# drowe67/pirip

Hardware: AMD Instinct MI355X
Metric: IQ Msamples/s demodulated (2-FSK Fs=240k Rs=10k); BER vs CPU ref (higher is better)
Workload: dtype f32

## Files before the change

### pirip_amd/csrc/fsk_demod_wave.hip

```cpp
#include <hip/hip_runtime.h>

#include <cmath>
#include <cstdio>
#include <cstdlib>
#include <type_traits>

#include "../../include/pirip_hip.h"
#include "demod_simd.hpp"
#include "fsk_device.hpp"

namespace pirip {

namespace {

constexpr int kWave = 64;

struct cf { float x, y; };

__device__ __forceinline__ float add_lane_up(float a, float b)
{
    float r;
    asm("v_add_f32_dpp %0, %1, %2 wave_shl:1 row_mask:0xf bank_mask:0xf bound_ctrl:0" : "=v"(r) : "v"(a), "v"(b));
    return r;
}
// ... 8 lines not shown
__device__ __forceinline__ float ubyte2(uint32_t v) { return (float)((v >> 16) & 0xffu); }
__device__ __forceinline__ float ubyte3(uint32_t v) { return (float)(v >> 24); }

__device__ __forceinline__ float llr_frame_gain_quick(int llr_map, float sig, float nse)
{
    const float a2 = sig - nse;
    if (!(a2 >= 0x1p-96f && a2 <= 0x1p126f)) return llr_frame_gain(llr_map, sig, nse);
    const float amp = sqrt_rn_normal<false>(a2);
    if (llr_map == kLlrRician) return (2.0f * amp) / nse;
    return (2.0f * (sig / nse)) / amp;
}
__device__ __forceinline__ unsigned sqrt_key(float x) { return __builtin_bit_cast(unsigned, x) - 1u; }
constexpr unsigned kSqrtLo = 0x0f800000u;
constexpr unsigned kQuickHi = 0x7c000000u;
__device__ __forceinline__ unsigned umin2(unsigned a, unsigned b) { return a < b ? a : b; }
__device__ __forceinline__ unsigned umin3(unsigned a, unsigned b, unsigned c)
{
    unsigned r;
    asm("v_min3_u32 %0, %1, %2, %3" : "=v"(r) : "v"(a), "v"(b), "v"(c));
    return r;
}

__device__ __forceinline__ v2f scale_lo(v2f h, v2f x)
{
    v2f r; asm("v_pk_mul_f32 %0, %1, %2 op_sel_hi:[0,1]" : "=v"(r) : "v"(h), "v"(x)); return r;
}
__device__ __forceinline__ v2f scale_hi(v2f h, v2f x)
{
    v2f r; asm("v_pk_mul_f32 %0, %1, %2 op_sel:[1,0] op_sel_hi:[1,1]" : "=v"(r) : "v"(h), "v"(x)); return r;
}
__device__ __forceinline__ float mag2(v2f w)
{
    v2f sq;
    asm("v_pk_mul_f32 %0, %1, %1" : "=v"(sq) : "v"(w));
    float r;
    asm("v_add_f32 %0, %1, %2" : "=v"(r) : "v"(sq.x), "v"(sq.y));
    return r;
}
__device__ __forceinline__ v2f smooth2(v2f sf, v2f mag, v2f k)
{
    v2f t;
    asm("v_pk_mul_f32 %0, %0, %3 op_sel_hi:[1,0]\n\t"
        "v_pk_mul_f32 %1, %2, %3 op_sel:[0,1] op_sel_hi:[1,1]\n\t"
        "v_pk_add_f32 %0, %0, %1"
        : "+v"(sf), "=&v"(t) : "v"(mag), "v"(k));
    return sf;
}

template <int B>
__device__ __forceinline__ uint32_t flag_mask_at(uint32_t flags)
{
    uint32_t r;
    asm("v_bfe_i32 %0, %1, %2, 1" : "=v"(r) : "v"(flags), "n"(B));
    return r;
}
__device__ __forceinline__ uint32_t flag_mask(uint32_t flags, int b)
{
    switch (b) {
    case 0: return flag_mask_at<0>(flags); case 1: return flag_mask_at<1>(flags); case 2: return flag_mask_at<2>(flags);
    case 3: return flag_mask_at<3>(flags); case 4: return flag_mask_at<4>(flags); case 5: return flag_mask_at<5>(flags);
    case 6: return flag_mask_at<6>(flags); default: return flag_mask_at<7>(flags);
    }
}

template <int FMT> struct InFmt;
template <> struct InFmt<PIRIP_IN_CU8_FSKDEMOD> { static constexpr int BPS = 2; static constexpr bool NEUTRAL_OK = true; static constexpr uint32_t NEUTRAL = 0x7F7F7F7Fu; };
template <> struct InFmt<PIRIP_IN_CU8_CSDR> { static constexpr int BPS = 2; static constexpr bool NEUTRAL_OK = false; static constexpr uint32_t NEUTRAL = 0x80808080u; };
template <> struct InFmt<PIRIP_IN_CS16> { static constexpr int BPS = 4; static constexpr bool NEUTRAL_OK = true; static constexpr uint32_t NEUTRAL = 0u; };
template <> struct InFmt<PIRIP_IN_CF32> { static constexpr int BPS = 8; static constexpr bool NEUTRAL_OK = true; static constexpr uint32_t NEUTRAL = 0u; };

__device__ __forceinline__ float cvt_s16(float x)
{
    const float hi = x * 0.00133514404296875f;
    return __builtin_fmaf(x, -0x1.e60f04p-20f, hi);
}
template <int FMT>
__device__ __forceinline__ v2f decode(const uint32_t *rw, int k)
{
    if (FMT == PIRIP_IN_CU8_FSKDEMOD || FMT == PIRIP_IN_CU8_CSDR) {
        const uint32_t v = rw[k >> 1];
        return cvt_u8_pair<FMT>(v2f{(k & 1) ? ubyte2(v) : ubyte0(v), (k & 1) ? ubyte3(v) : ubyte1(v)});
    } else if (FMT == PIRIP_IN_CS16) {
        const uint32_t v = rw[k];
        return v2f{cvt_s16((float)(short)(v & 0xffffu)), cvt_s16((float)((int)v >> 16))};
    } else {
        return v2f{__builtin_bit_cast(float, rw[2 * k]), __builtin_bit_cast(float, rw[2 * k + 1])};
    }
}
template <int FMT>
__device__ __forceinline__ v2f lds_sample(const unsigned char *p)
{
    if (FMT == PIRIP_IN_CU8_FSKDEMOD || FMT == PIRIP_IN_CU8_CSDR) {
        const uint32_t v = *(const uint16_t *)p;
        return cvt_u8_pair<FMT>(v2f{ubyte0(v), ubyte1(v)});
    } else if (FMT == PIRIP_IN_CS16) {
        const uint32_t v = *(const uint32_t *)p;
        return v2f{cvt_s16((float)(short)(v & 0xffffu)), cvt_s16((float)((int)v >> 16))};
    } else {
        const float2 v = *(const float2 *)p;
        return v2f{v.x, v.y};
    }
}

constexpr int cmax(int a, int b) { return a > b ? a : b; }

__device__ __forceinline__ float atan2_turns(float y, float x)
// ... 49 lines not shown
    static constexpr int NMEM = N + 2 * TS;
    static constexpr int Q = TS / 4;
    static constexpr int HIST = 2 * TS + Q;
    static constexpr int STEP = TS / P;
    static constexpr int NLANES = NSYM + 2;
    static constexpr int NFFT = (N - Q) / (NDFT / 2) - 1;
    static constexpr int GUARD_B = ((HIST * BPS + 15) / 16) * 16;
    static constexpr int SUP_B = (N + Q) * BPS;
    static constexpr int NDMA16 = SUP_B / 1024;
    static constexpr int NDMA4 = (SUP_B - NDMA16 * 1024 + 255) / 256;
    static constexpr bool DIRECT = FMT == PIRIP_IN_CF32 && NDFT >= 256;
    static constexpr int HEAD_B = 1024, DUMP_B = 256;
    static_assert(!DIRECT || ((TS + Q) * BPS <= HEAD_B && 3 * TS >= 2 * TS + Q), "the head holds blocks 0..2's new samples");
    static constexpr int RAW_B = DIRECT ? GUARD_B + HEAD_B + DUMP_B : GUARD_B + NDMA16 * 1024 + NDMA4 * 256;
    static constexpr int XPS256 = 16 * 17 * 8;
    static constexpr int XP_FFT_B = NDFT == 256 ? 4 * XPS256 : NDFT == 512 ? 4480 : 8 * 72 * 8;
    static constexpr int XP_B = cmax(cmax(XP_FFT_B, NDFT * 4), NDFT == 256 ? 64 * 20 * 4 : NDFT == 128 ? 8 * 136 * 4 : 0);
    static constexpr int TAIL_DW = HIST * BPS / 4;
    static constexpr int TRAILER_DW = GUARD_B / 4;
    static_assert((HIST * BPS) % 4 == 0 && (GUARD_B - HIST * BPS) % 4 == 0, "tail copies move whole dwords");
    static_assert(GUARD_B + (2 * M + 1) * 4 <= M * HIST * 8, "the state block holds the raw tail and its trailer");
    static constexpr int CHS = (BPS == 2) ? TS : (TS % 8 == 0 ? 8 : TS % 4 == 0 ? 4 : 2);
    static constexpr int CH_DW = CHS * BPS / 4;
    static_assert(TS % 2 == 0 && TS % P == 0 && P >= 4, "bad Ts / P");
    static_assert(NLANES <= kWave, "one lane per symbol block");
    static_assert((TS * BPS) % 16 == 0 && (CHS * BPS) % 16 == 0 && TS % CHS == 0, "block and chunk strides keep 16-byte alignment");
    static_assert((N + Q) / (NDFT / 2) - 1 == NFFT && N / (NDFT / 2) - 1 == NFFT, "numffts must not depend on nin");
    static_assert(NDFT == 256 ? (NFFT >= 4) : NDFT == 512 ? (NFFT % 2 == 0) : (NDFT == 128 && NFFT <= 8),
                  "FFT batches (Ndft = 256: the last batch of 4 may be partial; Ndft = 128: one batch of up to eight)");
    static_assert((NFFT - 1) * (NDFT / 2) + NDFT <= N - Q, "FFT windows stay inside the shortest frame");
    static_assert(M * P <= 48, "window prefix sums are kept in registers");
};

constexpr bool wave_plain_instance(int M, int TS, int P, int NDFT, int FMT, int WPS, bool FFT_FMA, bool MASK, int BAND)
{
    if (MASK && M == 4) return true;
    if (MASK && M == 2 && TS == 24 && FMT == PIRIP_IN_CU8_CSDR) return true;
    if (!MASK && M == 4 && FMT == PIRIP_IN_CF32 && (TS == 18 || TS == 10)) return true;
    return false;
}

constexpr bool wave_two_pass_argmax_instance(int M, int TS, int FMT, bool MASK, int BAND)
{
    if (MASK && M == 2 && TS == 24) return true;
    if (!MASK && M == 4 && (FMT == PIRIP_IN_CF32 || FMT == PIRIP_IN_CS16 || BAND == 4)) return true;
    return false;
}

constexpr bool wave_locked_paths_instance(int M, int TS, int P, int NDFT, int FMT, bool FFT_FMA, bool MASK, int BAND)
{
    return M == 2 && TS == 24 && P == 24 && NDFT == 256 && FMT == PIRIP_IN_CU8_FSKDEMOD && !FFT_FMA && !MASK && BAND == 0;
}

constexpr bool wave_packed_power_instance(int M, int TS, int P, int NDFT, int FMT, bool FFT_FMA, bool MASK, int BAND)
{
    return M == 2 && TS == 24 && P == 24 && NDFT == 256 && FMT == PIRIP_IN_CU8_FSKDEMOD && !FFT_FMA && !MASK;
}

constexpr bool wave_tail_prio_instance(int M, int TS, int P, int NDFT, int FMT, int WPS, bool FFT_FMA, bool MASK, int BAND)
{
    if (TS == 40 && M == 2 && FMT == PIRIP_IN_CS16 && !MASK) return false;
    if (TS == 40 && M == 4 && FMT == PIRIP_IN_CF32 && MASK) return false;
    if (TS == 8 && M == 2 && !MASK) return false;
    return true;
}

template <class C, int M> constexpr int wave_lds_bytes() { return C::RAW_B + C::XP_B; }

}

template <int M, int TS, int P, int NSYM, int NDFT, int FMT, int WPB, int WPS, bool FFT_FMA = false, bool MASK = false, int BAND = 0>
__global__ __launch_bounds__(kWave * WPB, WPS) void fsk_demod_wave_kernel(DemodArgs a_kernarg, int nstreams)
{
    constexpr bool INPLACE = TS == 10;
    constexpr bool PLAIN = wave_plain_instance(M, TS, P, NDFT, FMT, WPS, FFT_FMA, MASK, BAND);
    constexpr bool ARGMAX_SINGLE = !PLAIN && !wave_two_pass_argmax_instance(M, TS, FMT, MASK, BAND);
    constexpr bool TAIL_PRIO = wave_tail_prio_instance(M, TS, P, NDFT, FMT, WPS, FFT_FMA, MASK, BAND);
    constexpr bool PACKED_POWER = wave_packed_power_instance(M, TS, P, NDFT, FMT, FFT_FMA, MASK, BAND);
    static_assert(offsetof(DemodArgs, d) == 0, "the argument block is the first kernel argument");
    auto ap = [&]() {
        if constexpr (INPLACE) return (const __attribute__((address_space(4))) DemodArgs *)__builtin_amdgcn_kernarg_segment_ptr();
        else return (const DemodArgs *)&a_kernarg;
    }();
#define PIRIP_ARGS_REREAD() do { if constexpr (INPLACE) asm volatile("" : "+s"(ap)); } while (0)
#define a (*ap)
#define d (ap->d)
    static_assert(BAND == 0 || ((BAND == 2 || BAND == 4) && NDFT == 256 && !MASK), "band-only estimator: Ndft = 256, peak method, 32 or 64 bins");
    auto cmul = [](v2f x, v2f t) { return FFT_FMA ? rot_step(x, t) : cmul_x(x, t); };
    using C = WaveCfg<M, TS, P, NSYM, NDFT, FMT>;
    constexpr int N = C::N, NMEM = C::NMEM, HIST = C::HIST, STEP = C::STEP, Q = C::Q, BPS = C::BPS;
    constexpr int GUARD_B = C::GUARD_B;

    __shared__ __attribute__((aligned(16))) unsigned char s_raw[WPB][C::RAW_B];
    __shared__ __attribute__((aligned(16))) unsigned char s_xp[WPB][C::XP_B];
    constexpr int TAB_F = NDFT == 256 ? 12 * 16 * 4 : NDFT == 512 ? 8 * 16 * 2 + 12 * 32 * 2 : 8 * 16 * 2;
    __shared__ __attribute__((aligned(16))) float s_tab[TAB_F];
    __shared__ __attribute__((aligned(16))) float2 s_tph[P];
    __shared__ __attribute__((aligned(16))) float2 s_tgain[NSYM + 2];
    __shared__ float s_misc[WPB][3];
    extern __shared__ __attribute__((aligned(16))) float s_lnI0[];

    const int lane0 = threadIdx.x & (kWave - 1);
    const int wv = __builtin_amdgcn_readfirstlane(threadIdx.x >> 6);
    const int sid = blockIdx.x * WPB + wv;

    if (NDFT == 256) {
        for (int i = threadIdx.x; i < 12 * 16; i += kWave * WPB)
            ((float4 *)s_tab)[i] = ((const float4 *)a.t.fast_tab)[(i & 15) * 12 + (i >> 4)];
    } else {
        for (int i = threadIdx.x; i < TAB_F / 4; i += kWave * WPB) ((float4 *)s_tab)[i] = ((const float4 *)(a.t.fast_tab + NDFT))[i];
    }
    if constexpr (P <= 10) if (a.io.soft.llr) {
        if (a.io.soft.llr_map == kLlrRician) { for (int i = threadIdx.x; i < 258; i += kWave * WPB) s_lnI0[i] = a.io.soft.lnI0[i]; }
        else if (threadIdx.x < 20) {
            const int sg = threadIdx.x >> 2, cc = threadIdx.x & 3;
            const float c2 = sg == 0 ? 0.226f : sg == 1 ? 0.1245f : sg == 2 ? 0.0288f : sg == 3 ? 0.002f : 0.0f;
            const float c1 = sg == 0 ? 0.0125f : sg == 1 ? 0.2177f : sg == 2 ? 0.6314f : sg == 3 ? 0.9048f : 0.9867f;
            const float c0 = sg == 0 ? -0.0012f : sg == 1 ? -0.108f : sg == 2 ? -0.5645f : sg == 3 ? -1.2997f : -2.2053f;
            s_lnI0[threadIdx.x] = cc == 0 ? c2 : cc == 1 ? c1 : cc == 2 ? c0 : 0.0f;
        }
    }
    if (threadIdx.x < P) s_tph[threadIdx.x] = a.t.tph[threadIdx.x];
    if (threadIdx.x < NSYM + 2) s_tgain[threadIdx.x] = a.t.timing_rec[(threadIdx.x < NSYM + 1 ? threadIdx.x : 0) * P];
    __syncthreads();
    if (sid >= nstreams) return;
    if (a.io.seg && a.io.seg[sid].max_frames < 0) return;

    unsigned char *raw = s_raw[wv];
    unsigned char *xpb = s_xp[wv];

    uint32_t *st32 = (uint32_t *)(a.s.hist + (size_t)sid * M * HIST);
// ... 30 lines not shown

    float sc_norm_rx_timing, sc_ppm, sc_SNRest;
    int sc_nin;
    {
        const StreamScalars sc = a.s.scal[sid];
        sc_norm_rx_timing = sc.norm_rx_timing; sc_ppm = sc.ppm; sc_SNRest = sc.SNRest; sc_nin = sc.nin;
        if (lane0 == 0) { s_misc[wv][0] = sc.snr_est; s_misc[wv][1] = sc.EbNodB; s_misc[wv][2] = sc.v_est; }
    }

    int64_t seg_in = 0, out0 = 0, max_frames = a.io.max_frames;
    if (a.io.seg) {
        const SegDesc sd = a.io.seg[sid];
        seg_in = sd.in_off; out0 = sd.out_frame0; max_frames = sd.max_frames;
    }
    const uint8_t *in_base = a.io.in + (size_t)sid * a.io.in_stride + (size_t)seg_in * BPS;
    const int64_t nsamp = a.io.nsamp - seg_in;
    const __amdgpu_buffer_rsrc_t rsrc =
        __builtin_amdgcn_make_buffer_rsrc((void *)in_base, 0, (int)(uint32_t)(BPS * nsamp), 0x00020000);

    int nin = __builtin_amdgcn_readfirstlane(sc_nin);
    int64_t pos = 0, frame = 0;
    if (a.io.first) { pos = __builtin_amdgcn_readfirstlane(a.io.first[sid]); frame = pos ? 1 : 0; }
    const int64_t frame_first = frame;
    int last_freqi0 = 0, last_freqi1 = 0, last_freqi2 = 0, last_freqi3 = 0;

    uint32_t in_range = 0;
    if constexpr (!MASK && !PLAIN) {
#pragma unroll
        for (int b = 0; b < NB; b++) {
            const int sfi = (BAND && lane0 >= 16) ? -1 : own_sfi(lane0, b);
            if (sfi >= d.est_st && sfi < d.est_en) in_range |= 1u << b;
        }
    }
    constexpr bool FCACHE = WPS <= 3 && !PLAIN;
    constexpr bool KEEP_STEP = FCACHE && (M == 2 || WPS == 2);
    constexpr bool HIT_BRANCH = FCACHE && wave_locked_paths_instance(M, TS, P, NDFT, FMT, FFT_FMA, MASK, BAND);
    constexpr uint32_t kFcStale = 0x40000000u, kFcNever = 0x80000000u, kFcRan = 0x20000000u;
    static_assert(N + Q < 0x10000, "last frame's length leaves the flag bits free");
    v2f ph_c[FCACHE ? M : 1], step_c[KEEP_STEP ? M : 1];
    if constexpr (FCACHE) {
#pragma unroll
        for (int m = 0; m < M; m++) ph_c[m] = v2f{0.f, 0.f};
    }
    if constexpr (KEEP_STEP) {
#pragma unroll
        for (int m = 0; m < M; m++) step_c[m] = v2f{0.f, 0.f};
    }
    uint32_t ninp_fc = (uint32_t)ninp0 | (d.frame_cache ? kFcStale : kFcNever);
    constexpr bool LIVE_SLOTS = !PLAIN && NB == 4 && wave_locked_paths_instance(M, TS, P, NDFT, FMT, FFT_FMA, MASK, BAND);
    constexpr int NLIVE = 2;
    constexpr uint32_t kFcLowSlots = 0x10000000u;
    if constexpr (LIVE_SLOTS) {
        if (d.frame_cache && !__any((in_range >> NLIVE) != 0u)) ninp_fc |= kFcLowSlots;
    }

    typedef __attribute__((address_space(3))) void *lds_ptr;
    auto dma_frame = [&](int64_t p0) {
        const uint32_t goff = (uint32_t)__builtin_amdgcn_readfirstlane((int)(uint32_t)(p0 * BPS));
        if constexpr (C::DIRECT) {
            __builtin_amdgcn_raw_ptr_buffer_load_lds(rsrc, (lds_ptr)(raw + GUARD_B), 16, lane0 * 16, goff, 0, 0);
#pragma unroll
            for (int i = 0; i < (C::SUP_B + 8191) / 8192; i++)
                __builtin_amdgcn_raw_ptr_buffer_load_lds(rsrc, (lds_ptr)(raw + GUARD_B + C::HEAD_B), 4, lane0 * 128, goff + i * 8192, 0, 0);
            return;
        }
#pragma unroll
        for (int i = 0; i < C::NDMA16; i++)
            __builtin_amdgcn_raw_ptr_buffer_load_lds(rsrc, (lds_ptr)(raw + GUARD_B + i * 1024), 16, lane0 * 16, goff + i * 1024, 0, 0);
#pragma unroll
        for (int i = 0; i < C::NDMA4; i++)
            __builtin_amdgcn_raw_ptr_buffer_load_lds(rsrc, (lds_ptr)(raw + GUARD_B + C::NDMA16 * 1024 + i * 256), 4, lane0 * 4,
                                                     goff + C::NDMA16 * 1024 + i * 256, 0, 0);
    };
    constexpr bool SOFT_OK = P <= 10;
    uint32_t soft_carry = 0;
    int soft_cb = 0, soft_w = 0;
    uint32_t *words_o = nullptr;
    if constexpr (SOFT_OK) if (a.io.soft.llr) { words_o = a.io.soft.words + (size_t)sid * a.io.soft.words_stride + (a.io.soft.bit0 >> 5); }
    auto soft_append = [&](uint32_t W, int nb) {
        const uint32_t merged = soft_carry | (soft_cb ? (W >> soft_cb) : W);
        if (soft_cb + nb >= 32) {
            if (lane0 == 0) words_o[soft_w] = merged;
            soft_w++;
            soft_carry = soft_cb ? (W << (32 - soft_cb)) : 0u;
            soft_cb = soft_cb + nb - 32;
        } else { soft_carry = merged; soft_cb += nb; }
    };
    constexpr int NBITS = NSYM * (M == 2 ? 1 : 2);
    wave_lds_sync();
    dma_frame(pos);
    if constexpr (TAIL_PRIO) {
        auto tp = (const __attribute__((address_space(4))) DemodArgs *)__builtin_amdgcn_kernarg_segment_ptr();
        if (sid / WPB >= tp->first_tail_block) __builtin_amdgcn_s_setprio(1);
    }
    PIRIP_T_DECL;

    while (frame < max_frames && pos + nin <= nsamp) {
        PIRIP_ARGS_REREAD();
        const int nold = NMEM - nin;
        PIRIP_T_MARK(7);
        asm volatile("s_waitcnt vmcnt(0)" ::: "memory");
        wave_lds_sync();
        PIRIP_T_MARK(0);
        const unsigned char *smp = raw + GUARD_B;
        const uint32_t goff_frame = (uint32_t)__builtin_amdgcn_readfirstlane((int)(uint32_t)(pos * BPS));
        auto fft_in = [&](const unsigned char *p) -> v2f {
            if constexpr (C::DIRECT && BPS == 8) {
                const auto v = __builtin_amdgcn_raw_buffer_load_b64(rsrc, (int)(p - smp), (int)goff_frame, 0);
                return __builtin_bit_cast(v2f, v);
            } else if constexpr (C::DIRECT) {
                const uint32_t v = (uint32_t)__builtin_amdgcn_raw_buffer_load_b32(rsrc, (int)(p - smp), (int)goff_frame, 0);
                return v2f{cvt_s16((float)(short)(v & 0xffffu)), cvt_s16((float)((int)v >> 16))};
            } else return lds_sample<FMT>(p);
        };
        const v2f ktc{d.one_minus_tc, d.tc};
        if constexpr (NDFT == 256) {
            PIRIP_PHASE_LANE(lane);
            const int grp = lane >> 4, e16 = lane & 15;
            const float4 *ftab = (const float4 *)s_tab + e16;
            constexpr int XPS = C::XPS256;
            float4 tabv[12];
#pragma unroll
            for (int i = 0; i < 12; i++) tabv[i] = ftab[16 * i];
#pragma unroll 1
            for (int bt = 0; bt < (C::NFFT + 3) / 4; bt++) {
                int jj = 4 * bt + grp;
                if (C::NFFT % 4) jj = jj < C::NFFT ? jj : C::NFFT - 1;
                const int ga = e16 >> 2, gb = e16 & 3;
                const int base = ga + 4 * gb;
                const unsigned char *src = smp + BPS * ((NDFT / 2) * jj + base);
                v2f W[16];
                v2f hann2[8];
                {
                    const float4 h0 = tabv[0], h1 = tabv[1], h2 = tabv[2], h3 = tabv[3];
                    hann2[0] = v2f{h0.x, h0.y}; hann2[1] = v2f{h0.z, h0.w}; hann2[2] = v2f{h1.x, h1.y}; hann2[3] = v2f{h1.z, h1.w};
                    hann2[4] = v2f{h2.x, h2.y}; hann2[5] = v2f{h2.z, h2.w}; hann2[6] = v2f{h3.x, h3.y}; hann2[7] = v2f{h3.z, h3.w};
                }
#pragma unroll
                for (int t = 0; t < 16; t++) {
                    const v2f x = fft_in(src + 16 * BPS * t);
                    const int c = t & 3, dd = t >> 2;
                    W[4 * c + dd] = (t & 1) ? scale_hi(hann2[t >> 1], x) : scale_lo(hann2[t >> 1], x);
                }
#pragma unroll
                for (int c = 0; c < 4; c++) bfly4(W[4 * c], W[4 * c + 1], W[4 * c + 2], W[4 * c + 3]);
                bfly4(W[0], W[4], W[8], W[12]);
#pragma unroll
                for (int k = 1; k < 4; k++) {
                    v2f f1 = cmul(W[4 + k], v2f{a.tw_s2[6 * (k - 1) + 0], a.tw_s2[6 * (k - 1) + 1]});
                    v2f f2 = cmul(W[8 + k], v2f{a.tw_s2[6 * (k - 1) + 2], a.tw_s2[6 * (k - 1) + 3]});
                    v2f f3 = cmul(W[12 + k], v2f{a.tw_s2[6 * (k - 1) + 4], a.tw_s2[6 * (k - 1) + 5]});
                    bfly4(W[k], f1, f2, f3);
                    W[4 + k] = f1; W[8 + k] = f2; W[12 + k] = f3;
                }
                {
                    float2 *xp = (float2 *)(xpb + grp * XPS);
#pragma unroll
                    for (int e = 0; e < 16; e++) xp[e16 * 17 + e] = make_float2(W[e].x, W[e].y);
                    wave_lds_sync();
#pragma unroll
                    for (int g = 0; g < 16; g++) { const float2 v = xp[g * 17 + e16]; W[g] = v2f{v.x, v.y}; }
                }
                {
                    const float4 c4 = tabv[4], c5 = tabv[5];
                    const v2f tw3[3] = {v2f{c4.x, c4.y}, v2f{c4.z, c4.w}, v2f{c5.x, c5.y}};
#pragma unroll
                    for (int aa = 0; aa < 4; aa++) {
                        v2f f1 = cmul(W[4 * aa + 1], tw3[0]);
                        v2f f2 = cmul(W[4 * aa + 2], tw3[1]);
                        v2f f3 = cmul(W[4 * aa + 3], tw3[2]);
                        bfly4(W[4 * aa], f1, f2, f3);
                        W[4 * aa + 1] = f1; W[4 * aa + 2] = f2; W[4 * aa + 3] = f3;
                    }
                }
#pragma unroll
                for (int b = 0; b < (BAND ? BAND : 4); b++) {
                    const float *trow = (const float *)(ftab);
                    auto tf = [&](int f) { const float4 c = tabv[f >> 2]; return (f & 3) == 0 ? c.x : (f & 3) == 1 ? c.y : (f & 3) == 2 ? c.z : c.w; };
                    (void)trow;
                    const v2f t1{tf(22 + 6 * b), tf(23 + 6 * b)}, t2{tf(24 + 6 * b), tf(25 + 6 * b)}, t3{tf(26 + 6 * b), tf(27 + 6 * b)};
                    v2f f1 = cmul(W[4 + b], t1);
                    v2f f2 = cmul(W[8 + b], t2);
                    v2f f3 = cmul(W[12 + b], t3);
                    bfly4(W[b], f1, f2, f3);
                    W[4 + b] = f1; W[8 + b] = f2; W[12 + b] = f3;
                }
                wave_lds_sync();
                if constexpr (BAND != 0) {
                    float m2b[BAND], rb[BAND];
                    unsigned kmin = 0xffffffffu;
#pragma unroll
                    for (int b = 0; b < BAND; b++) { m2b[b] = mag2(W[b]); kmin = umin2(kmin, fbits(m2b[b])); }
                    if (__all(kmin >= kSqrtLo)) {
#pragma unroll
                        for (int b = 0; b < BAND; b++) rb[b] = sqrt_rn_normal<FMT != PIRIP_IN_CF32, true>(m2b[b]);
                    } else {
                        kmin = 0xffffffffu;
#pragma unroll
                        for (int b = 0; b < BAND; b++) kmin = umin2(kmin, sqrt_key(m2b[b]));
                        if (__all(kmin >= kSqrtLo - 1u)) {
#pragma unroll
                            for (int b = 0; b < BAND; b++) rb[b] = sqrt_rn_normal<FMT != PIRIP_IN_CF32>(m2b[b]);
                        } else {
#pragma unroll
// ... 250 lines not shown
                    for (int q0 = 0; q0 < 4; q0++) { const float2 v = x2[q0 * 40 + L5]; Y[4 * q0 + j1] = v2f{v.x, v.y}; }
                }
                float mag[16];
#pragma unroll
                for (int j1 = 0; j1 < 4; j1++) {
                    const float2 t1 = s_p3[(3 * j1 + 0) * 32 + L5], t2 = s_p3[(3 * j1 + 1) * 32 + L5], t3 = s_p3[(3 * j1 + 2) * 32 + L5];
                    v2f f0 = Y[j1];
                    v2f f1 = cmul(Y[4 + j1], v2f{t1.x, t1.y});
                    v2f f2 = cmul(Y[8 + j1], v2f{t2.x, t2.y});
                    v2f f3 = cmul(Y[12 + j1], v2f{t3.x, t3.y});
                    bfly4(f0, f1, f2, f3);
                    mag[j1] = mag2(f0); mag[j1 + 4] = mag2(f1); mag[j1 + 8] = mag2(f2); mag[j1 + 12] = mag2(f3);
                }
                float A[8], B[8];
                unsigned kmin = 0xffffffffu;
#pragma unroll
                for (int u = 0; u < 8; u++) {
                    A[u] = mag[u]; B[u] = mag[u + 8];
                    asm volatile("s_nop 1\n\tv_permlane32_swap_b32 %0, %1" : "+v"(A[u]), "+v"(B[u]));
                    kmin = umin3(kmin, fbits(A[u]), fbits(B[u]));
                }
                if (__all(kmin >= kSqrtLo)) {
#pragma unroll
                    for (int u = 0; u < 8; u++) { A[u] = sqrt_rn_normal<FMT != PIRIP_IN_CF32, true>(A[u]); B[u] = sqrt_rn_normal<FMT != PIRIP_IN_CF32, true>(B[u]); }
                } else {
                    kmin = 0xffffffffu;
#pragma unroll
                    for (int u = 0; u < 8; u++) kmin = umin3(kmin, sqrt_key(A[u]), sqrt_key(B[u]));
                    if (__all(kmin >= kSqrtLo - 1u)) {
#pragma unroll
                        for (int u = 0; u < 8; u++) { A[u] = sqrt_rn_normal<FMT != PIRIP_IN_CF32>(A[u]); B[u] = sqrt_rn_normal<FMT != PIRIP_IN_CF32>(B[u]); }
                    } else {
#pragma unroll
                        for (int u = 0; u < 8; u++) { A[u] = sqrtf(A[u]); B[u] = sqrtf(B[u]); __builtin_amdgcn_sched_barrier(0); }
                    }
                }
#pragma unroll
                for (int u = 0; u < 8; u += 2) {
                    v2f sp{Sf[u], Sf[u + 1]};
                    sp = smooth2(sp, v2f{A[u], A[u + 1]}, ktc);
                    sp = smooth2(sp, v2f{B[u], B[u + 1]}, ktc);
                    Sf[u] = sp.x; Sf[u + 1] = sp.y;
                }
                wave_lds_sync();
            }
        }

        __builtin_amdgcn_sched_barrier(0);
        PIRIP_T_MARK(1);
        int freqi[M];
#pragma unroll
        for (int m = 0; m < M; m++) freqi[m] = 0;
        int bb = 0;
        if constexpr (MASK) {
            PIRIP_PHASE_LANE(lane);
            float *sfl = (float *)xpb;
#pragma unroll
            for (int b = 0; b < NOWN; b++) sfl[own_sfi(lane, b)] = Sf[b];
            wave_lds_sync();
            float best = 0.0f; int ib = d.est_st;
            for (int b = d.est_st + lane; b < d.est_en - d.mask_len; b += kWave) {
                float corr = 0.0f;
                for (int k = 0; k < d.n_teeth; k++) corr += sfl[b + a.t.teeth[k]];
                if (corr > best) { best = corr; ib = b; }
            }
            wave_argmax<ARGMAX_SINGLE>(best, ib);
            bb = ib;
            wave_lds_sync();
        } else {
            PIRIP_PHASE_LANE(lane);
            if constexpr (LIVE_SLOTS) {
                const int f_zero = d.f_zero;
                auto pick = [&](auto nbl_c) __attribute__((always_inline)) {
                    constexpr int NBL = decltype(nbl_c)::value;
                    float w[NBL];
                    int sfi[NBL];
#pragma unroll
                    for (int b = 0; b < NBL; b++) {
                        sfi[b] = (BAND && lane >= 16) ? -1 : own_sfi(lane, b);
                        w[b] = __builtin_bit_cast(float, fbits(Sf[b]) & flag_mask(in_range, b));
                    }
#pragma unroll
                    for (int m = 0; m < M; m++) {
                        float best = 0.0f; int ib = 0;
#pragma unroll
                        for (int b = 0; b < NBL; b++)
                            if (w[b] > best) { best = w[b]; ib = sfi[b]; }
                        wave_argmax<ARGMAX_SINGLE>(best, ib);
                        int f_min = ib - f_zero; f_min = f_min < 0 ? 0 : f_min;
                        int f_max = ib + f_zero; f_max = f_max > NDFT ? NDFT : f_max;
#pragma unroll
                        for (int b = 0; b < NBL; b++) if (sfi[b] >= f_min && sfi[b] < f_max) w[b] = 0.0f;
                        freqi[m] = ib - NDFT / 2;
                    }
                };
                if (ninp_fc & kFcLowSlots) pick(std::integral_constant<int, NLIVE>{});
                else pick(std::integral_constant<int, NB>{});
            } else {
                float w[NB];
                int sfi[NB];
                static_assert(NB <= 8, "one flag bit per owned bin");
#pragma unroll
                for (int b = 0; b < NB; b++) {
                    sfi[b] = (BAND && lane >= 16) ? -1 : own_sfi(lane, b);
                    if constexpr (PLAIN) w[b] = (sfi[b] >= d.est_st && sfi[b] < d.est_en) ? Sf[b] : 0.0f;
                    else w[b] = __builtin_bit_cast(float, fbits(Sf[b]) & flag_mask(in_range, b));
                }
#pragma unroll
                for (int m = 0; m < M; m++) {
                    float best = 0.0f; int ib = 0;
#pragma unroll
                    for (int b = 0; b < NB; b++)
                        if (w[b] > best) { best = w[b]; ib = sfi[b]; }
                    wave_argmax<ARGMAX_SINGLE>(best, ib);
                    int f_min = ib - d.f_zero; f_min = f_min < 0 ? 0 : f_min;
                    int f_max = ib + d.f_zero; f_max = f_max > NDFT ? NDFT : f_max;
#pragma unroll
                    for (int b = 0; b < NB; b++) if (sfi[b] >= f_min && sfi[b] < f_max) w[b] = 0.0f;
                    freqi[m] = ib - NDFT / 2;
                }
            }
#pragma unroll
            for (int x = 1; x < M; x++)
#pragma unroll
                for (int y = x; y > 0; y--)
                    if (freqi[y] < freqi[y - 1]) { const int t = freqi[y]; freqi[y] = freqi[y - 1]; freqi[y - 1] = t; }
        }
        constexpr int LOG2N = NDFT == 128 ? 7 : NDFT == 256 ? 8 : 9;
        uint32_t dthv[M];
        int tix[M];
#pragma unroll
        for (int m = 0; m < M; m++) {
            if constexpr (MASK) { dthv[m] = a.t.mask_dtheta[bb * M + m]; tix[m] = bb * M + m; }
            else { dthv[m] = (uint32_t)freqi[m] << (32 - LOG2N); tix[m] = freqi[m] + NDFT / 2; }
        }

        auto phasor = [&](uint32_t th) {
            const float2 w = a.t.tw[th >> (32 - LOG2N)];
            float pc = w.x, ps = -w.y;
            if constexpr (MASK) {
                const float bl = (float)(th & ((1u << (32 - LOG2N)) - 1u)) * 1.4629180792671596e-9f;
                const float b2 = bl * bl;
                const float cb = 1.0f - b2 * (0.5f - b2 * (1.0f / 24.0f));
                const float sb = bl * (1.0f - b2 * ((1.0f / 6.0f) - b2 * (1.0f / 120.0f)));
                const float c2 = pc * cb - ps * sb, s2 = ps * cb + pc * sb;
                pc = c2; ps = s2;
            }
            return make_float2(pc, ps);
        };
        __builtin_amdgcn_sched_barrier(0);
        PIRIP_T_MARK(2);
        v2f fi[M][P];
        v2f tot[M];
        {
            PIRIP_PHASE_LANE(lane);
            const int lb = lane < C::NLANES ? lane : C::NLANES - 1;
            const int boff = GUARD_B + (TS * lb - nold) * BPS;
            const int al = (GUARD_B - nold * BPS) & 15;
            v2f ph[M], dph[M], acc[M];
            v2f sw_ph[M], sw_dph[M];
            const int n0 = TS * lb - nold + 1;
            const int nold_blk = nold - TS * lb;
            const bool oldl = nold_blk > 0;
            const int ninp = (int)(ninp_fc & 0xffffu);
            const int zero_blk = ninp ? 0 : nold_blk;
            uint32_t moved = (uint32_t)(nin ^ N) | (uint32_t)(ninp ^ N);
#pragma unroll
            for (int m = 0; m < M; m++) moved |= (uint32_t)(tix[m] ^ tixp[m]);
            static_assert(Q > 0 && Q < TS, "a block changes oscillators at sample Ts/4 or Ts - Ts/4 only: never where nold_blk is a multiple of Ts");
            const bool hit = FCACHE && (moved | (ninp_fc & (kFcStale | kFcNever))) == 0;
            if (hit) {
#pragma unroll
                for (int m = 0; m < M; m++) {
                    if constexpr (KEEP_STEP) dph[m] = step_c[m];
                    else { const float2 stn = a.t.osc_step[tix[m]]; dph[m] = v2f{stn.x, stn.y}; }
                    if constexpr (FCACHE) ph[m] = ph_c[m];
                    if constexpr (!HIT_BRANCH) { sw_ph[m] = dph[m]; sw_dph[m] = dph[m]; }
                }
            } else {
#pragma unroll
                for (int m = 0; m < M; m++) {
                    const float2 stn = a.t.osc_step[tix[m]], stp = a.t.osc_step[tixp[m]];
                    const float dn = a.t.osc_drift[tix[m]].x, dp = a.t.osc_drift[tixp[m]].x;
                    const uint32_t th = (uint32_t)n0 * (oldl ? dthp[m] : dthv[m]);
                    const float g = 1.0f + (oldl ? dp * (float)(ninp + n0) : dn * (float)n0);
                    const float2 pcs = phasor(th);
                    ph[m] = v2f{pcs.x * g, pcs.y * g};
                    dph[m] = oldl ? v2f{stp.x, stp.y} : v2f{stn.x, stn.y};
                    const float2 p1 = phasor(dthv[m]);
                    const float g1 = 1.0f + dn;
                    sw_ph[m] = v2f{p1.x * g1, p1.y * g1};
                    sw_dph[m] = v2f{stn.x, stn.y};
                    if constexpr (FCACHE) ph_c[m] = ph[m];
                    if constexpr (KEEP_STEP) step_c[m] = sw_dph[m];
                }
            }
            if constexpr (KEEP_STEP) {
#pragma unroll
                for (int m = 0; m < M; m++) sw_dph[m] = step_c[m];
            }
            ninp_fc = (uint32_t)nin | (PLAIN ? 0u : kFcRan) | (ninp_fc & (kFcNever | kFcLowSlots)) | (FCACHE ? ((moved + (kFcStale - 1u)) & kFcStale) : 0u);
#pragma unroll
            for (int m = 0; m < M; m++) acc[m] = v2f{0.f, 0.f};
#pragma unroll
            for (int c = 0; c < TS / C::CHS; c++) {
                uint32_t rw[C::CH_DW];
                if (C::DIRECT && lb >= 3) {
#pragma unroll
                    for (int i = 0; i < C::CH_DW / 4; i++) {
                        const auto v = __builtin_amdgcn_raw_buffer_load_b128(rsrc, (TS * lb - nold) * BPS + c * C::CHS * BPS + 16 * i, (int)goff_frame, 0);
                        const uint4 u = __builtin_bit_cast(uint4, v);
                        rw[4 * i] = u.x; rw[4 * i + 1] = u.y; rw[4 * i + 2] = u.z; rw[4 * i + 3] = u.w;
                    }
                } else {
                    const unsigned char *bp = raw + boff + c * C::CHS * BPS;
                    if (al == 0) {
#pragma unroll
                        for (int i = 0; i < C::CH_DW / 4; i++) {
                            const uint4 v = ((const uint4 *)bp)[i];
                            rw[4 * i] = v.x; rw[4 * i + 1] = v.y; rw[4 * i + 2] = v.z; rw[4 * i + 3] = v.w;
                        }
// ... 32 lines not shown
                    if (M == 2) asm volatile("" : "+v"(nacc[0]), "+v"(nacc[M - 1]));
                    else asm volatile("" : "+v"(nacc[0]), "+v"(nacc[1]), "+v"(nacc[M - 2]), "+v"(nacc[M - 1]));
#pragma unroll
                    for (int m = 0; m < M; m++) {
                        if (k % STEP == 0) fi[m][k / STEP] = acc[m];
                        acc[m] = nacc[m];
                    }
                    if ((kk & 3) == 3) __builtin_amdgcn_sched_barrier(0);
                }
            }
#pragma unroll
            for (int m = 0; m < M; m++) tot[m] = acc[m];
        }
        PIRIP_PHASE_LANE(lane);
        if constexpr (C::DIRECT) {
            asm volatile("s_waitcnt lgkmcnt(0)" ::: "memory");
            wave_lds_sync();
            const uint32_t toff = (uint32_t)__builtin_amdgcn_readfirstlane((int)(uint32_t)((pos + nin - HIST) * BPS));
#pragma unroll
            for (int i = 0; i < (C::TAIL_DW + kWave - 1) / kWave; i++)
                if (lane + i * kWave < C::TAIL_DW)
                    __builtin_amdgcn_raw_ptr_buffer_load_lds(rsrc, (lds_ptr)(raw + GUARD_B - HIST * BPS + i * 256), 4, lane * 4, toff + i * 256, 0, 0);
        } else {
            const uint32_t *tsrc = (const uint32_t *)(raw + GUARD_B + (nin - HIST) * BPS);
            uint32_t *tdst = (uint32_t *)(raw + GUARD_B - HIST * BPS);
            uint32_t tv[(C::TAIL_DW + kWave - 1) / kWave];
#pragma unroll
            for (int i = 0; i < (C::TAIL_DW + kWave - 1) / kWave; i++) tv[i] = tsrc[lane + i * kWave < C::TAIL_DW ? lane + i * kWave : 0];
#pragma unroll
            for (int i = 0; i < (C::TAIL_DW + kWave - 1) / kWave; i++) if (lane + i * kWave < C::TAIL_DW) tdst[lane + i * kWave] = tv[i];
        }
        asm volatile("s_waitcnt lgkmcnt(0)" ::: "memory");
        wave_lds_sync();
        PIRIP_T_MARK(3);
        dma_frame(pos + nin);
#pragma unroll
        for (int m = 0; m < M; m++) { dthp[m] = dthv[m]; tixp[m] = tix[m]; }

        float tcr = 0.f, tci = 0.f;
        {
            v2f prpi{0.f, 0.f};
            v2f ft{0.f, 0.f};
            constexpr int GROUP = PACKED_POWER ? 4 : 1;
            static_assert(P % GROUP == 0, "whole groups of window starts");
#pragma unroll
            for (int q = 0; q < P; q++) {
                v2f sq;
                const v2f tp = *(const v2f *)&s_tph[q];
                if (PACKED_POWER && q % GROUP == 0) __builtin_amdgcn_sched_barrier(0);
#pragma unroll
                for (int m = 0; m < M; m++) {
                    const v2f own = fi[m][q];
                    v2f w0;
                    w0.x = add_lane_up(own.x, tot[m].x - own.x);
                    w0.y = add_lane_up(own.y, tot[m].y - own.y);
                    fi[m][q] = w0;
                    if constexpr (PACKED_POWER) {
                        if (m == 0) asm("v_pk_mul_f32 %0, %1, %1" : "=v"(sq) : "v"(w0));
                        else asm("v_pk_fma_f32 %0, %1, %1, %0" : "+v"(sq) : "v"(w0));
                    } else {
                        if (m == 0) asm("v_mul_f32 %0, %1, %1\n\tv_fma_f32 %0, %2, %2, %0" : "=&v"(ft.x) : "v"(w0.y), "v"(w0.x));
                        else { float t2; asm("v_mul_f32 %0, %2, %2\n\tv_fma_f32 %0, %3, %3, %0\n\tv_add_f32 %1, %1, %0" : "=&v"(t2), "+v"(ft.x) : "v"(w0.y), "v"(w0.x)); }
                    }
                }
                if constexpr (PACKED_POWER) asm("v_add_f32 %0, %1, %2" : "=v"(ft.x) : "v"(sq.x), "v"(sq.y));
                asm("v_pk_fma_f32 %0, %1, %2, %0 op_sel_hi:[0,1,1]" : "+v"(prpi) : "v"(ft), "v"(tp));
                if constexpr (GROUP == 1) asm volatile("" : "+v"(prpi), "+v"(fi[0][q]), "+v"(fi[M - 1][q]));
                else if (q % GROUP == GROUP - 1) {
                    asm volatile("" : "+v"(prpi));
#pragma unroll
                    for (int k = q + 1 - GROUP; k <= q; k++) asm volatile("" : "+v"(fi[0][k]), "+v"(fi[M - 1][k]));
                }
            }
            const float pr = prpi.x, pi = prpi.y;
            if (lane <= NSYM) {
                const float2 tgain = s_tgain[lane];
                tcr = pr * tgain.x - pi * tgain.y;
                tci = pr * tgain.y + pi * tgain.x;
            }
            tcr = wave_sum(tcr); tci = wave_sum(tci);
        }

        PIRIP_T_MARK(4);
        PIRIP_ARGS_REREAD();
        const int frame_bytes = d.pack_bits ? (NBITS + 7) / 8 : NBITS;
        const size_t orow = (size_t)(frame + out0);
        uint8_t *bits_o = a.io.bits ? a.io.bits + (size_t)sid * a.io.bits_stride + orow * frame_bytes : nullptr;
        float *filt_o = a.io.filt ? a.io.filt + (size_t)sid * a.io.filt_stride + orow * M * NSYM : nullptr;
        float *stats_o = a.io.stats ? a.io.stats + (size_t)sid * a.io.stats_stride + orow * PIRIP_STATS_PER_FRAME : nullptr;
        const bool bad = isnan(tcr) || isnan(tci);
        int nin_next = nin;
        if (!bad) {
            const float norm_rx_timing = FMT == PIRIP_IN_CF32 ? atan2f(tci, tcr) * 0.15915494309189535f : atan2_turns(tci, tcr);
            const float rx_timing = norm_rx_timing * (float)P;
            const float d_norm = norm_rx_timing - sc_norm_rx_timing;
            sc_norm_rx_timing = norm_rx_timing;
            if (fabsf(d_norm) < 0.2f) {
                const float x6 = 1e6f * d_norm;
                float appm;
                if (PACKED_POWER && !(ninp_fc & kFcNever) && __all(fabsf(x6) >= 0x1p-125f || fbits(x6) == 0u)) appm = div_rn_const<NSYM>(x6);
                else appm = x6 / (float)NSYM;
                sc_ppm = (0.9f * sc_ppm) + (0.1f * appm);
            }
            nin_next = N;
            if (!d.burst_mode) {
                if (norm_rx_timing > 0.25f) nin_next = N + Q;
                else if (norm_rx_timing < -0.25f) nin_next = N - Q;
            }
// ... 404 lines not shown
```

Measured before the change: 384,200.

## Confirm previous frame's tone picks cheaply before running full argmax search

For the locked M=2 cu8 instance with frame cache, the code first checks whether the two tones chosen in the previous frame are still the unique maxima. It reads their smoothed magnitudes with readlane and counts, by ballot, how many bins reach them, using zone masks cached in spare in_range bits. If both remain unique, it reuses the previous picks and skips the iterative argmax and the sort. Otherwise it runs the normal pick and records new zone bits. The cost is extra ballots and readlanes on every frame, plus added register pressure and branch complexity.

```diff
diff --git a/pirip_amd/csrc/fsk_demod_wave.hip b/pirip_amd/csrc/fsk_demod_wave.hip
--- a/pirip_amd/csrc/fsk_demod_wave.hip
+++ b/pirip_amd/csrc/fsk_demod_wave.hip
@@ -84,6 +84,12 @@
 {
     uint32_t r;
     asm("v_bfe_i32 %0, %1, %2, 1" : "=v"(r) : "v"(flags), "n"(B));
+    return r;
+}
+__device__ __forceinline__ uint32_t flag_mask_s(uint32_t flags, int b)
+{
+    uint32_t r;
+    asm("v_bfe_i32 %0, %1, %2, 1" : "=v"(r) : "v"(flags), "s"(b));
     return r;
 }
 __device__ __forceinline__ uint32_t flag_mask(uint32_t flags, int b)
@@ -239,6 +245,11 @@
     return M == 2 && TS == 24 && P == 24 && NDFT == 256 && FMT == PIRIP_IN_CU8_FSKDEMOD && !FFT_FMA && !MASK && BAND == 0;
 }
 
+constexpr bool wave_confirmed_pick_instance(int M, int TS, int P, int NDFT, int FMT, bool FFT_FMA, bool MASK, int BAND)
+{
+    return wave_locked_paths_instance(M, TS, P, NDFT, FMT, FFT_FMA, MASK, BAND);
+}
+
 constexpr bool wave_packed_power_instance(int M, int TS, int P, int NDFT, int FMT, bool FFT_FMA, bool MASK, int BAND)
 {
     return M == 2 && TS == 24 && P == 24 && NDFT == 256 && FMT == PIRIP_IN_CU8_FSKDEMOD && !FFT_FMA && !MASK;
@@ -401,6 +412,8 @@
     if constexpr (LIVE_SLOTS) {
         if (d.frame_cache && !__any((in_range >> NLIVE) != 0u)) ninp_fc |= kFcLowSlots;
     }
+    constexpr bool CONFIRM = LIVE_SLOTS && FCACHE && wave_confirmed_pick_instance(M, TS, P, NDFT, FMT, FFT_FMA, MASK, BAND);
+    constexpr int kZoneBit = 8;
 
     typedef __attribute__((address_space(3))) void *lds_ptr;
     auto dma_frame = [&](int64_t p0) {
@@ -854,6 +867,7 @@
 #pragma unroll
         for (int m = 0; m < M; m++) freqi[m] = 0;
         int bb = 0;
+        [[maybe_unused]] uint32_t tone_moved = 0;
         if constexpr (MASK) {
             PIRIP_PHASE_LANE(lane);
             float *sfl = (float *)xpb;
@@ -896,8 +910,58 @@
                         freqi[m] = ib - NDFT / 2;
                     }
                 };
-                if (ninp_fc & kFcLowSlots) pick(std::integral_constant<int, NLIVE>{});
-                else pick(std::integral_constant<int, NB>{});
+                if constexpr (CONFIRM) {
+                    bool confirmed = false;
+                    if ((ninp_fc & (kFcStale | kFcNever | kFcLowSlots)) == kFcLowSlots) {
+                        const int bin_a = tixp[0] ^ (NDFT / 2), bin_b = tixp[1] ^ (NDFT / 2);
+                        const int ln_a = __builtin_amdgcn_readfirstlane((bin_a & 15) | ((bin_a >> 6) << 4));
+                        const int ln_b = __builtin_amdgcn_readfirstlane((bin_b & 15) | ((bin_b >> 6) << 4));
+                        const float w0 = __builtin_bit_cast(float, fbits(Sf[0]) & flag_mask(in_range, 0));
+                        const float w1 = __builtin_bit_cast(float, fbits(Sf[1]) & flag_mask(in_range, 1));
+                        const uint32_t a0 = (uint32_t)__builtin_amdgcn_readlane((int)fbits(w0), ln_a), a1 = (uint32_t)__builtin_amdgcn_readlane((int)fbits(w1), ln_a);
+                        const uint32_t b0 = (uint32_t)__builtin_amdgcn_readlane((int)fbits(w0), ln_b), b1 = (uint32_t)__builtin_amdgcn_readlane((int)fbits(w1), ln_b);
+                        const uint32_t va = (bin_a & 16) ? a1 : a0, vb = (bin_b & 16) ? b1 : b0;
+                        const bool b_hi = vb > va;
+                        const uint32_t v_hi = b_hi ? vb : va, v_lo = b_hi ? va : vb;
+                        const int hi = b_hi ? tixp[1] : tixp[0], lo = b_hi ? tixp[0] : tixp[1];
+                        int f_min = hi - f_zero; f_min = f_min < 0 ? 0 : f_min;
+                        int f_max = hi + f_zero; f_max = f_max > NDFT ? NDFT : f_max;
+                        const float f_hi = __builtin_bit_cast(float, v_hi), f_lo = __builtin_bit_cast(float, v_lo);
+                        const int n_hi = __builtin_popcountll(__ballot(w0 >= f_hi)) + __builtin_popcountll(__ballot(w1 >= f_hi));
+                        const int zoff = kZoneBit + (b_hi ? NLIVE : 0);
+                        const float z0 = __builtin_bit_cast(float, fbits(Sf[0]) & flag_mask_s(in_range, zoff));
+                        const float z1 = __builtin_bit_cast(float, fbits(Sf[1]) & flag_mask_s(in_range, zoff + 1));
+                        const int n_lo = __builtin_popcountll(__ballot(z0 >= f_lo)) + __builtin_popcountll(__ballot(z1 >= f_lo));
+                        confirmed = ((bin_a | bin_b) & 32) == 0 && va != vb && v_lo != 0u && (lo < f_min || lo >= f_max) && n_hi == 1 && n_lo == 1;
+                    }
+                    if (confirmed) {
+#pragma unroll
+                        for (int m = 0; m < M; m++) freqi[m] = tixp[m] - NDFT / 2;
+                        tone_moved = 0u;
+                    } else {
+                        if (ninp_fc & kFcLowSlots) pick(std::integral_constant<int, NLIVE>{});
+                        else pick(std::integral_constant<int, NB>{});
+                        if (freqi[1] < freqi[0]) { const int t = freqi[1]; freqi[1] = freqi[0]; freqi[0] = t; }
+                        tone_moved = (uint32_t)((freqi[0] + NDFT / 2) ^ tixp[0]) | (uint32_t)((freqi[1] + NDFT / 2) ^ tixp[1]);
+                        uint32_t zb = 0;
+#pragma unroll
+                        for (int m = 0; m < M; m++) {
+                            const int ib = freqi[m] + NDFT / 2;
+                            int z_min = ib - f_zero; z_min = z_min < 0 ? 0 : z_min;
+                            int z_max = ib + f_zero; z_max = z_max > NDFT ? NDFT : z_max;
+#pragma unroll
+                            for (int b = 0; b < NLIVE; b++) {
+                                const int sfi = own_sfi(lane, b);
+                                if (!(sfi >= z_min && sfi < z_max)) zb |= 1u << (kZoneBit + NLIVE * m + b);
+                            }
+                        }
+                        const uint32_t live = in_range & ((1u << NLIVE) - 1u);
+                        in_range = (in_range & 0xffu) | (zb & ((live << kZoneBit) | (live << (kZoneBit + NLIVE))));
+                    }
+                } else {
+                    if (ninp_fc & kFcLowSlots) pick(std::integral_constant<int, NLIVE>{});
+                    else pick(std::integral_constant<int, NB>{});
+                }
             } else {
                 float w[NB];
                 int sfi[NB];
@@ -922,11 +986,13 @@
                     freqi[m] = ib - NDFT / 2;
                 }
             }
-#pragma unroll
-            for (int x = 1; x < M; x++)
-#pragma unroll
-                for (int y = x; y > 0; y--)
-                    if (freqi[y] < freqi[y - 1]) { const int t = freqi[y]; freqi[y] = freqi[y - 1]; freqi[y - 1] = t; }
+            if constexpr (!CONFIRM) {
+#pragma unroll
+                for (int x = 1; x < M; x++)
+#pragma unroll
+                    for (int y = x; y > 0; y--)
+                        if (freqi[y] < freqi[y - 1]) { const int t = freqi[y]; freqi[y] = freqi[y - 1]; freqi[y - 1] = t; }
+            }
         }
         constexpr int LOG2N = NDFT == 128 ? 7 : NDFT == 256 ? 8 : 9;
         uint32_t dthv[M];
@@ -967,8 +1033,11 @@
             const int ninp = (int)(ninp_fc & 0xffffu);
             const int zero_blk = ninp ? 0 : nold_blk;
             uint32_t moved = (uint32_t)(nin ^ N) | (uint32_t)(ninp ^ N);
-#pragma unroll
-            for (int m = 0; m < M; m++) moved |= (uint32_t)(tix[m] ^ tixp[m]);
+            if constexpr (CONFIRM) moved |= tone_moved;
+            else {
+#pragma unroll
+                for (int m = 0; m < M; m++) moved |= (uint32_t)(tix[m] ^ tixp[m]);
+            }
             static_assert(Q > 0 && Q < TS, "a block changes oscillators at sample Ts/4 or Ts - Ts/4 only: never where nold_blk is a multiple of Ts");
             const bool hit = FCACHE && (moved | (ninp_fc & (kFcStale | kFcNever))) == 0;
             if (hit) {
```

New measurement: 387,500 (median of 6 runs). About the same (+0.9%).

## Share converted input samples across overlapping FFT frames via LDS in cu8 path

Applied to the files above, without the earlier changes.

For the M=2, TS=24, cu8 instance, each FFT group now converts only half of its 16 input samples. The other half, which overlaps the next 50%-overlapped frame, is exchanged through the transpose LDS area, so each sample is decoded once instead of twice. The stage-2 twiddles are hoisted from kernel arguments into registers, and the q==0 lane-shift in the power loop is replaced by a direct copy of the total. This adds an LDS round trip and a wave sync per batch, raises register pressure, and relies on static asserts that reading past the frame stays in range.

```diff
diff --git a/pirip_amd/csrc/fsk_demod_wave.hip b/pirip_amd/csrc/fsk_demod_wave.hip
--- a/pirip_amd/csrc/fsk_demod_wave.hip
+++ b/pirip_amd/csrc/fsk_demod_wave.hip
@@ -244,6 +244,11 @@
     return M == 2 && TS == 24 && P == 24 && NDFT == 256 && FMT == PIRIP_IN_CU8_FSKDEMOD && !FFT_FMA && !MASK;
 }
 
+constexpr bool wave_shared_convert_instance(int M, int TS, int P, int NDFT, int FMT, bool FFT_FMA, bool MASK, int BAND)
+{
+    return M == 2 && TS == 24 && P == 24 && NDFT == 256 && FMT == PIRIP_IN_CU8_FSKDEMOD && !FFT_FMA && !MASK;
+}
+
 constexpr bool wave_tail_prio_instance(int M, int TS, int P, int NDFT, int FMT, int WPS, bool FFT_FMA, bool MASK, int BAND)
 {
     if (TS == 40 && M == 2 && FMT == PIRIP_IN_CS16 && !MASK) return false;
@@ -264,6 +269,7 @@
     constexpr bool ARGMAX_SINGLE = !PLAIN && !wave_two_pass_argmax_instance(M, TS, FMT, MASK, BAND);
     constexpr bool TAIL_PRIO = wave_tail_prio_instance(M, TS, P, NDFT, FMT, WPS, FFT_FMA, MASK, BAND);
     constexpr bool PACKED_POWER = wave_packed_power_instance(M, TS, P, NDFT, FMT, FFT_FMA, MASK, BAND);
+    constexpr bool SHARED_CONVERT = wave_shared_convert_instance(M, TS, P, NDFT, FMT, FFT_FMA, MASK, BAND);
     static_assert(offsetof(DemodArgs, d) == 0, "the argument block is the first kernel argument");
     auto ap = [&]() {
         if constexpr (INPLACE) return (const __attribute__((address_space(4))) DemodArgs *)__builtin_amdgcn_kernarg_segment_ptr();
@@ -400,6 +406,12 @@
     constexpr uint32_t kFcLowSlots = 0x10000000u;
     if constexpr (LIVE_SLOTS) {
         if (d.frame_cache && !__any((in_range >> NLIVE) != 0u)) ninp_fc |= kFcLowSlots;
+    }
+
+    v2f tw2v[SHARED_CONVERT ? 9 : 1];
+    if constexpr (SHARED_CONVERT) {
+#pragma unroll
+        for (int i = 0; i < 9; i++) { tw2v[i] = v2f{a.tw_s2[2 * i], a.tw_s2[2 * i + 1]}; asm volatile("" : "+v"(tw2v[i])); }
     }
 
     typedef __attribute__((address_space(3))) void *lds_ptr;
@@ -484,20 +496,60 @@
                     hann2[0] = v2f{h0.x, h0.y}; hann2[1] = v2f{h0.z, h0.w}; hann2[2] = v2f{h1.x, h1.y}; hann2[3] = v2f{h1.z, h1.w};
                     hann2[4] = v2f{h2.x, h2.y}; hann2[5] = v2f{h2.z, h2.w}; hann2[6] = v2f{h3.x, h3.y}; hann2[7] = v2f{h3.z, h3.w};
                 }
-#pragma unroll
-                for (int t = 0; t < 16; t++) {
-                    const v2f x = fft_in(src + 16 * BPS * t);
-                    const int c = t & 3, dd = t >> 2;
-                    W[4 * c + dd] = (t & 1) ? scale_hi(hann2[t >> 1], x) : scale_lo(hann2[t >> 1], x);
+                if constexpr (SHARED_CONVERT) {
+                    constexpr int CVS = 144;
+                    static_assert(C::NFFT % 4 == 0 && !C::DIRECT && NDFT == 256, "whole batches of four FFTs over staged samples");
+                    static_assert(5 * CVS * 8 <= C::XP_B, "the conversion area fits the transpose area: no new LDS");
+                    static_assert((4 * ((C::NFFT + 3) / 4) + 1) * (NDFT / 2) <= N - Q, "round B stays inside the shortest frame");
+                    float2 *cv = (float2 *)xpb;
+                    v2f xin[16];
+#pragma unroll
+                    for (int t = 0; t < 8; t++) xin[t] = lds_sample<FMT>(src + 16 * BPS * t);
+                    v2f xb[2];
+                    {
+                        const unsigned char *sb = smp + BPS * ((NDFT / 2) * (4 * bt + 4) + lane);
+#pragma unroll
+                        for (int h = 0; h < 2; h++) xb[h] = lds_sample<FMT>(sb + BPS * 64 * h);
+                    }
+#pragma unroll
+                    for (int t = 0; t < 8; t++) cv[grp * CVS + base + 16 * t] = make_float2(xin[t].x, xin[t].y);
+#pragma unroll
+                    for (int h = 0; h < 2; h++) cv[4 * CVS + lane + 64 * h] = make_float2(xb[h].x, xb[h].y);
+                    wave_lds_sync();
+#pragma unroll
+                    for (int t = 0; t < 8; t++) { const float2 v = cv[(grp + 1) * CVS + base + 16 * t]; xin[8 + t] = v2f{v.x, v.y}; }
+#pragma unroll
+                    for (int half = 0; half < 2; half++) {
+                        __builtin_amdgcn_sched_barrier(0);
+#pragma unroll
+                        for (int t = 8 * half; t < 8 * half + 8; t++) {
+                            const int c = t & 3, dd = t >> 2;
+                            W[4 * c + dd] = (t & 1) ? scale_hi(hann2[t >> 1], xin[t]) : scale_lo(hann2[t >> 1], xin[t]);
+                        }
+                    }
+                } else {
+#pragma unroll
+                    for (int t = 0; t < 16; t++) {
+                        const v2f x = fft_in(src + 16 * BPS * t);
+                        const int c = t & 3, dd = t >> 2;
+                        W[4 * c + dd] = (t & 1) ? scale_hi(hann2[t >> 1], x) : scale_lo(hann2[t >> 1], x);
+                    }
                 }
 #pragma unroll
                 for (int c = 0; c < 4; c++) bfly4(W[4 * c], W[4 * c + 1], W[4 * c + 2], W[4 * c + 3]);
                 bfly4(W[0], W[4], W[8], W[12]);
 #pragma unroll
                 for (int k = 1; k < 4; k++) {
-                    v2f f1 = cmul(W[4 + k], v2f{a.tw_s2[6 * (k - 1) + 0], a.tw_s2[6 * (k - 1) + 1]});
-                    v2f f2 = cmul(W[8 + k], v2f{a.tw_s2[6 * (k - 1) + 2], a.tw_s2[6 * (k - 1) + 3]});
-                    v2f f3 = cmul(W[12 + k], v2f{a.tw_s2[6 * (k - 1) + 4], a.tw_s2[6 * (k - 1) + 5]});
+                    v2f t1, t2, t3;
+                    if constexpr (SHARED_CONVERT) { t1 = tw2v[3 * (k - 1)]; t2 = tw2v[3 * (k - 1) + 1]; t3 = tw2v[3 * (k - 1) + 2]; }
+                    else {
+                        t1 = v2f{a.tw_s2[6 * (k - 1) + 0], a.tw_s2[6 * (k - 1) + 1]};
+                        t2 = v2f{a.tw_s2[6 * (k - 1) + 2], a.tw_s2[6 * (k - 1) + 3]};
+                        t3 = v2f{a.tw_s2[6 * (k - 1) + 4], a.tw_s2[6 * (k - 1) + 5]};
+                    }
+                    v2f f1 = cmul(W[4 + k], t1);
+                    v2f f2 = cmul(W[8 + k], t2);
+                    v2f f3 = cmul(W[12 + k], t3);
                     bfly4(W[k], f1, f2, f3);
                     W[4 + k] = f1; W[8 + k] = f2; W[12 + k] = f3;
                 }
@@ -1107,8 +1159,12 @@
                 for (int m = 0; m < M; m++) {
                     const v2f own = fi[m][q];
                     v2f w0;
-                    w0.x = add_lane_up(own.x, tot[m].x - own.x);
-                    w0.y = add_lane_up(own.y, tot[m].y - own.y);
+                    if (SHARED_CONVERT && q == 0) {
+                        w0 = tot[m];
+                    } else {
+                        w0.x = add_lane_up(own.x, tot[m].x - own.x);
+                        w0.y = add_lane_up(own.y, tot[m].y - own.y);
+                    }
                     fi[m][q] = w0;
                     if constexpr (PACKED_POWER) {
                         if (m == 0) asm("v_pk_mul_f32 %0, %1, %1" : "=v"(sq) : "v"(w0));
```

Result: no change. 389,600 before, 386,600 after (-0.8%).
